# tictacmenthe/F2CNN

Measured on AMD Instinct MI355X. Metric: audio-seconds/sec through filterbank+envelope (HIP, 1 MI355X per rank); the +CNN figure of BASELINE's metric is value_with_cnn / blocks.cfg4, higher is better.
Workload: dtype f64 filter state + f64 utterance FFT + f32 row FFT; 1 GPU; cfg3: filterbank + Hilbert envelope + 50 Hz LPF in one call (f32 FFT), batch of 1000 x 1 s utterances per GPU, 128 channels, ENV1 (float64) out; channels=128, lpf_hz=50, launch_batch=1000, outputs_resident_in_hbm=True, parallelism=utterance-sharded x1, no collective, utterances_sent_back_by_the_accuracy_guard=0

## Files before the change

### f2cnn_amd/csrc/f2_api.hip

```cpp
#include "f2_internal.h"

char g_f2_err[512] = {0};

int f2_fail(f2_ctx* ctx, int code, const char* fmt, ...) {
    char* dst = ctx ? ctx->err : g_f2_err;
    va_list ap;
    va_start(ap, fmt);
    vsnprintf(dst, 512, fmt, ap);
    va_end(ap);
    return code;
}

int f2_reserve(f2_ctx* ctx, f2_scratch& s, size_t bytes) {
    if (bytes <= s.bytes) return F2_OK;
    if (s.ptr) {
        F2_HIP(ctx, hipStreamSynchronize(ctx->stream));
        F2_HIP(ctx, hipFree(s.ptr));
        s.ptr = nullptr;
        s.bytes = 0;
    }
    size_t want = (bytes + 255) & ~size_t(255);
    hipError_t e = hipMalloc(&s.ptr, want);
    if (e != hipSuccess) {
        s.ptr = nullptr;
// ... 170 lines not shown
    }
    *count = n;
    return F2_OK;
}

int f2_ctx_create(int device, f2_ctx** out) {
    if (!out) return f2_fail(nullptr, F2_ERR_INVALID, "ctx out pointer is NULL");
    *out = nullptr;
    int n = 0;
    hipError_t e = hipGetDeviceCount(&n);
    if (e != hipSuccess || n <= 0)
        return f2_fail(nullptr, F2_ERR_HIP, "no HIP device available (%s)",
                       e != hipSuccess ? hipGetErrorString(e) : "device count is 0");
    if (device < 0 || device >= n) return f2_fail(nullptr, F2_ERR_INVALID, "device %d out of range [0,%d)", device, n);
    f2_ctx* ctx = new f2_ctx();
    ctx->device = device;
    e = hipSetDevice(device);
    if (e == hipSuccess) e = hipStreamCreateWithFlags(&ctx->stream, hipStreamNonBlocking);
    hipDeviceProp_t prop;
    if (e == hipSuccess) e = hipGetDeviceProperties(&prop, device);
    if (e == hipSuccess) e = hipHostMalloc((void**)&ctx->host_flags, 64, hipHostMallocDefault);
    if (e != hipSuccess) {
        f2_fail(nullptr, F2_ERR_HIP, "context setup on device %d -> %s", device, hipGetErrorString(e));
        delete ctx;
        return F2_ERR_HIP;
    }
    ctx->num_cus = prop.multiProcessorCount;
    if (strncmp(prop.gcnArchName, "gfx950", 6) != 0) {
        f2_fail(nullptr, F2_ERR_UNSUPPORTED, "device %d is %s; this library is built for gfx950 only", device,
                prop.gcnArchName);
        (void)hipStreamDestroy(ctx->stream);
        (void)hipHostFree(ctx->host_flags);
        delete ctx;
        return F2_ERR_UNSUPPORTED;
    }
    int rc = f2_reserve(ctx, ctx->flags, 64);
    if (rc != F2_OK) {
        memcpy(g_f2_err, ctx->err, sizeof(g_f2_err));
        (void)hipStreamDestroy(ctx->stream);
        (void)hipHostFree(ctx->host_flags);
        delete ctx;
        return rc;
    }
    *out = ctx;
    return F2_OK;
}

int f2_ctx_destroy(f2_ctx* ctx) {
    if (!ctx) return F2_OK;
    (void)hipSetDevice(ctx->device);
    (void)hipStreamSynchronize(ctx->stream);
    f2_scratch* all[] = {&ctx->coefs, &ctx->offsets, &ctx->stage_in, &ctx->stage_out, &ctx->stage_aux,
                         &ctx->work,  &ctx->work2,   &ctx->xbuf,      &ctx->flags,    &ctx->gather_log, &ctx->dense_in,
                         &ctx->stamps, &ctx->noise_wave, &ctx->noise_meta, &ctx->acc_meta, &ctx->score_meta};
    for (f2_scratch* s : all)
        if (s->ptr) (void)hipFree(s->ptr);
    for (auto& v : ctx->prof)
        for (auto& pr : v) {
            (void)hipEventDestroy(pr.first);
            (void)hipEventDestroy(pr.second);
        }
    for (hipEvent_t e : ctx->prof_pool) (void)hipEventDestroy(e);
    for (auto& prec : ctx->tw)
        for (f2_scratch& s : prec)
            if (s.ptr) (void)hipFree(s.ptr);
    for (auto& prec : ctx->tw_large)
        for (f2_scratch& s : prec)
            if (s.ptr) (void)hipFree(s.ptr);
    for (f2_scratch& s : ctx->tw_p3)
        if (s.ptr) (void)hipFree(s.ptr);
    for (f2_scratch& s : ctx->tw_fl)
        if (s.ptr) (void)hipFree(s.ptr);
    for (f2_scratch& s : ctx->tw_split)
        if (s.ptr) (void)hipFree(s.ptr);
    for (f2_scratch* sc : {&ctx->tw_pair[0], &ctx->tw_pair[1], &ctx->pair_list[0], &ctx->pair_list[1]})
        if (sc->ptr) (void)hipFree(sc->ptr);
    if (ctx->work3.ptr) (void)hipFree(ctx->work3.ptr);
    if (ctx->k1_states.ptr) (void)hipFree(ctx->k1_states.ptr);
    if (ctx->k1_mtab.ptr) (void)hipFree(ctx->k1_mtab.ptr);
    if (ctx->k1_order.ptr) (void)hipFree(ctx->k1_order.ptr);
    if (ctx->handoff.ptr) (void)hipFree(ctx->handoff.ptr);
    if (ctx->handoff_off.ptr) (void)hipFree(ctx->handoff_off.ptr);
    for (auto& t : ctx->spec_tabs)
        for (f2_scratch* sc : {&t.hu, &t.e, &t.lgroup, &t.e64})
            if (sc->ptr) (void)hipFree(sc->ptr);
    for (f2_scratch* sc : {&ctx->spec_x, &ctx->spec_rho, &ctx->spec_xpart, &ctx->spec_meta, &ctx->spec_uflag, &ctx->spec_lptab})
        if (sc->ptr) (void)hipFree(sc->ptr);
    for (auto& prec : ctx->tw_sp)
        for (f2_scratch& sc : prec)
            if (sc.ptr) (void)hipFree(sc.ptr);
    for (auto& sp : ctx->up_inflight) (void)hipEventDestroy(sp.done);
    for (auto& b : ctx->up_big) {
        if (b.ptr) (void)hipHostFree(b.ptr);
        (void)hipEventDestroy(b.done);
    }
    if (ctx->up_ring) (void)hipHostFree(ctx->up_ring);
    if (ctx->host_flags) (void)hipHostFree(ctx->host_flags);
    if (ctx->own_stream && ctx->stream) (void)hipStreamDestroy(ctx->stream);
    delete ctx;
    return F2_OK;
}

int f2_ctx_synchronize(f2_ctx* ctx) {
    F2_CHECK(nullptr, ctx, F2_ERR_INVALID, "ctx is NULL");
    F2_HIP(ctx, hipStreamSynchronize(ctx->stream));
    return F2_OK;
}

int f2_ctx_set_stream(f2_ctx* ctx, void* hip_stream) {
    F2_CHECK(nullptr, ctx, F2_ERR_INVALID, "ctx is NULL");
    F2_HIP(ctx, hipStreamSynchronize(ctx->stream));
    if (ctx->own_stream && ctx->stream) F2_HIP(ctx, hipStreamDestroy(ctx->stream));
    if (hip_stream) {
        ctx->stream = (hipStream_t)hip_stream;
        ctx->own_stream = false;
    } else {
        F2_HIP(ctx, hipStreamCreateWithFlags(&ctx->stream, hipStreamNonBlocking));
        ctx->own_stream = true;
    }
    return F2_OK;
}

void* f2_ctx_get_stream(f2_ctx* ctx) { return ctx ? (void*)ctx->stream : nullptr; }

const char* f2_last_error(f2_ctx* ctx) { return ctx ? ctx->err : g_f2_err; }

namespace {
struct opt_entry {
    const char* key;
    int f2_ctx::*ifield;
    float f2_ctx::*ffield;
    double lo, hi;
};
const opt_entry kOptions[] = {
    {"spectral", &f2_ctx::opt_spectral, nullptr, 0, 1},
    {"spectral_tol", nullptr, &f2_ctx::opt_spectral_tol, 0, 1},
    {"spectral_min_rows", &f2_ctx::opt_spectral_min_rows, nullptr, 0, 1 << 30},
    {"spectral_min_pad", &f2_ctx::opt_spectral_min_pad, nullptr, -1, 1 << 16},
    {"spectral_guard_dump", &f2_ctx::opt_spectral_guard_dump, nullptr, 0, 1},
    {"k1_split", &f2_ctx::opt_k1_split, nullptr, -1, 64},
    {"k1_queue", &f2_ctx::opt_k1_queue, nullptr, -1, 1},
    {"k1_qwaves", &f2_ctx::opt_k1_qwaves, nullptr, 0, 1 << 20},
    {"env_pair", &f2_ctx::opt_env_pair, nullptr, 0, 1},
    {"env_plan4", &f2_ctx::opt_env_plan4, nullptr, 0, 1},
    {"cnn_f16x3", &f2_ctx::opt_cnn_f16x3, nullptr, 0, 1},
    {"cnn_bf16x3", &f2_ctx::opt_cnn_f16x3, nullptr, 0, 1},
    {"cnn_ws", &f2_ctx::opt_cnn_ws, nullptr, 0, 1},
    {"cnn_ws_dense", &f2_ctx::opt_cnn_ws_dense, nullptr, 0, 1},
    {"gather_blocked", &f2_ctx::opt_gather_blocked, nullptr, 0, 1},
};
const opt_entry* find_option(const char* key) {
    if (!key) return nullptr;
    for (const opt_entry& e : kOptions)
        if (strcmp(e.key, key) == 0) return &e;
    return nullptr;
}
}

int f2_ctx_set_option(f2_ctx* ctx, const char* key, double value) {
    F2_CHECK(nullptr, ctx, F2_ERR_INVALID, "ctx is NULL");
    const opt_entry* e = find_option(key);
    F2_CHECK(ctx, e, F2_ERR_INVALID, "unknown option '%s'", key ? key : "(null)");
    F2_CHECK(ctx, value >= e->lo && value <= e->hi, F2_ERR_INVALID, "option %s: %g outside [%g, %g]", key, value, e->lo, e->hi);
    if (e->ifield) {
        F2_CHECK(ctx, value == (double)(int)value, F2_ERR_INVALID, "option %s takes an integer", key);
        ctx->*(e->ifield) = (int)value;
    } else {
// ... 475 lines not shown
```

### f2cnn_amd/csrc/f2_internal.h

```cpp
#pragma once
#include <hip/hip_runtime.h>

#include <cstdarg>
#include <cstdint>
#include <cstdio>
#include <cstring>
#include <mutex>
#include <string>
#include <utility>
#include <vector>

#include "../../include/f2cnn_hip.h"

struct f2_scratch {
    void* ptr = nullptr;
    size_t bytes = 0;
};

struct f2_spec_tables {
    int log2h = 0, C = 0;
    std::vector<double> coefs;
    int64_t tpitch = 0;
    f2_scratch hu, e, lgroup, e64;
};
#define F2_SPECTRAL_MIN_LOG2H 12
#define F2_SPECTRAL_MAX_LOG2H 15

struct f2_ctx {
    int device = 0;
    hipStream_t stream = nullptr;
    bool own_stream = true;
    int num_cus = 0;
    char err[512] = {0};
    f2_scratch coefs;
    f2_scratch offsets;
    f2_scratch stage_in;
    f2_scratch stage_out;
    f2_scratch stage_aux;
    f2_scratch work;
    f2_scratch work2;
    f2_scratch xbuf;
    f2_scratch dense_in;
    f2_scratch noise_wave;
    f2_scratch noise_meta;
    f2_scratch acc_meta;
    f2_scratch score_meta;
    f2_scratch gather_log;
    f2_scratch tw[2][16];
    f2_scratch tw_fl[16];
    f2_scratch tw_p3[2];
    f2_scratch tw_large[2][24];
    f2_scratch tw_split[24];
    std::vector<int> pair_list_host[2];
    f2_scratch tw_pair[2], pair_list[2];
    f2_scratch work3;
    f2_scratch handoff, handoff_off;
    std::vector<int64_t> handoff_off_host;
    f2_scratch k1_states, k1_mtab;
    f2_scratch k1_order;
    int k1_mtab_L = 0;
    std::vector<double> k1_mtab_coefs;
    std::vector<int64_t> offsets_host;
    std::vector<double> coefs_host;
    bool prof_on = false;
    struct prof_span {
        hipEvent_t first, second;
        bool closed;
    };
    std::vector<prof_span> prof[F2_K_COUNT];
    std::vector<hipEvent_t> prof_pool;
    std::vector<f2_spec_tables> spec_tabs;
    f2_scratch spec_x, spec_rho;
    f2_scratch spec_xpart;
    f2_scratch spec_meta, spec_uflag;
    f2_scratch spec_gdump;
    size_t spec_gdump_rows = 0;
    std::vector<int> spec_meta_host;
    int spec_coefs_ok = -1;
    int spec_min_pad = 64;
    size_t spec_last_B = 0;
    f2_scratch tw_sp[2][16];
    f2_scratch spec_lptab;
    double spec_lptab_a1 = 0.0;
    int spec_lptab_nt = 0;
    int opt_spectral = 1;
    int opt_spectral_min_rows = 4096;
    float opt_spectral_tol = 4e-6f;
    int opt_spectral_min_pad = -1;
    int opt_spectral_guard_dump = 0;
    int opt_k1_split = -1;
    int opt_k1_queue = -1;
    int opt_k1_qwaves = 0;
    int opt_env_pair = 1;
    int opt_cnn_f16x3 = 1;
    int opt_cnn_ws = 1;
    int opt_cnn_ws_dense = 1;
    int opt_gather_blocked = 1;
    int opt_env_plan4 = 0;
    char* up_ring = nullptr;
    size_t up_cap = 0, up_head = 0;
    struct up_span {
        size_t begin, end;
        hipEvent_t done;
    };
    std::vector<up_span> up_inflight;
    struct up_side {
// ... 221 lines not shown
```

### f2cnn_amd/csrc/f2_spectral.hip

```cpp
#define f2fft f2fft_sp
#undef F2_PLAN13_PASSES
#define F2_PLAN13_PASSES 4
#include <algorithm>
#include <cmath>
#include <complex>
#include <thread>

#include "f2_fft_lds.h"

using namespace f2fft;

namespace {

typedef float f2_f4 __attribute__((ext_vector_type(4)));
constexpr int SPEC_GB = 16;

constexpr int KS_CGROUP = 32;
constexpr int KS_CGROUP_LONG = 8;
constexpr int KS_STORE_AUX = 2;
typedef unsigned int f2_u4 __attribute__((ext_vector_type(4)));
typedef unsigned int f2_u2 __attribute__((ext_vector_type(2)));
__device__ __forceinline__ __amdgpu_buffer_rsrc_t row_buffer(double* y, int n) {
    return __builtin_amdgcn_make_buffer_rsrc(y, 0, n * 8, 0x00020000);
}
// ... 593 lines not shown
    constexpr int D = 1 << LOGD;
    constexpr int NT = threads_for<double, LOG2H>();
    constexpr int H = 1 << LOG2H;
    constexpr int CS = cpad_size(H);
    constexpr int R0 = 1 << plan_bits(LOG2H, 0);
    constexpr int NB0 = H / R0;
    constexpr int ITER0 = (NB0 + NT - 1) / NT;
    constexpr int PT = plan_points_per_thread(LOG2H, NT);
    constexpr bool FULL0 = NB0 % NT == 0;
    __shared__ __attribute__((aligned(16))) cpx<double> lds[CS];
    constexpr int TWL = plan_tw_lds_count(LOG2H);
    __shared__ __attribute__((aligned(16))) cpx<double> twl[TWL > 0 ? TWL : 1];
    const cpx<double>* __restrict__ V = tw + plan_tw_total(LOG2H);
    const int tid = threadIdx.x;
    const int ul = blockIdx.x >> LOGD, ph = blockIdx.x & (D - 1);
    const int b = ulist[ul];
    const int64_t off = offsets[b];
    const int n = (int)(offsets[b + 1] - off);
    const WaveT* __restrict__ x = wave + off;
    for (int i = tid; i < TWL; i += NT) twl[i] = tw[plan_tw_offset(LOG2H, 1) + i];
    cpx<double> v[PT];
#pragma unroll
    for (int i = 0; i < ITER0; ++i) {
        const int bf = tid + i * NT;
        if (FULL0 || bf < NB0) {
#pragma unroll
            for (int j = 0; j < R0; ++j) {
                const int i0 = D * 2 * (bf + j * NB0) + ph, i1 = i0 + D;
                v[i * R0 + j] = {i0 < n ? (double)x[i0] : 0.0, i1 < n ? (double)x[i1] : 0.0};
            }
        }
    }
    fft_all<double, LOG2H, false, PT, NT, false>(lds, tw, twl, tid, v);
    cpx<float>* __restrict__ Xo = X + (size_t)ul * xpitch;
    cpx<double>* __restrict__ Xp = Xpart + (size_t)blockIdx.x * (H + 1);
    for (int k = 1 + tid; k <= H / 2; k += NT) {
        const cpx<double> zk = lds[cpad(k)], zh = lds[cpad(H - k)];
        const cpx<double> e = {0.5 * (zk.re + zh.re), 0.5 * (zk.im - zh.im)};
        const cpx<double> o = {0.5 * (zk.im + zh.im), -0.5 * (zk.re - zh.re)};
        const cpx<double> w = V[k];
        const cpx<double> wo = {o.re * w.re - o.im * w.im, o.re * w.im + o.im * w.re};
        if constexpr (LOGD == 0) {
            Xo[k] = {(float)(e.re + wo.re), (float)(e.im + wo.im)};
            Xo[H - k] = {(float)(e.re - wo.re), (float)(-(e.im - wo.im))};
        } else {
            Xp[k] = {e.re + wo.re, e.im + wo.im};
            Xp[H - k] = {e.re - wo.re, -(e.im - wo.im)};
        }
    }
    if (tid == 0) {
        const cpx<double> z0 = lds[cpad(0)];
        if constexpr (LOGD == 0) {
            Xo[0] = {(float)(z0.re + z0.im), 0.f};
            Xo[H] = {(float)(z0.re - z0.im), 0.f};
        } else {
            Xp[0] = {z0.re + z0.im, 0.0};
            Xp[H] = {z0.re - z0.im, 0.0};
        }
    }
}

template <int LOG2HS, int LOGD>
__global__ __launch_bounds__(256) void k_spectrum_combine(const cpx<double>* __restrict__ Xpart, const cpx<double>* __restrict__ e64,
                                                          cpx<float>* __restrict__ X, int64_t xpitch) {
    constexpr int D = 1 << LOGD, HS = 1 << LOG2HS, H = D * HS, M = 2 * H;
    const int ul = blockIdx.y;
    const int k = blockIdx.x * 256 + threadIdx.x;
    if (k > H) return;
    const int kk = k & (2 * HS - 1);
    double re = 0.0, im = 0.0;
#pragma unroll
    for (int ph = 0; ph < D; ++ph) {
        const cpx<double>* __restrict__ Xp = Xpart + ((size_t)ul * D + ph) * (HS + 1);
        cpx<double> xp = kk <= HS ? Xp[kk] : Xp[2 * HS - kk];
        if (kk > HS) xp.im = -xp.im;
        const cpx<double> w = e64[(ph * k) & (M - 1)];
        re += xp.re * w.re - xp.im * w.im;
        im += xp.re * w.im + xp.im * w.re;
    }
    X[(size_t)ul * xpitch + k] = {(float)re, (float)im};
}

constexpr int TAIL_TB = 32;
constexpr int TAIL_WAVES = 4;

template <typename WaveT>
__global__ __launch_bounds__((64 * TAIL_WAVES)) void k_tail_state(const WaveT* __restrict__ wave, const int64_t* __restrict__ offsets,
                                                                const double* __restrict__ coefs, int C, int groups,
                                                                const int* __restrict__ ulist, int nutt,
                                                                const int* __restrict__ Lgroup, float* __restrict__ rho,
                                                                double two_over_m) {
    __shared__ double xss[TAIL_WAVES][TAIL_TB];
    const int lane = threadIdx.x & 63;
    const int wid = __builtin_amdgcn_readfirstlane(threadIdx.x >> 6);
    const int unit = blockIdx.x * TAIL_WAVES + wid;
    if (unit >= nutt * groups) return;
    const int ul = unit / groups, g = unit - ul * groups;
    const int b = ulist[ul];
    const int64_t off = offsets[b];
    const int64_t N = offsets[b + 1] - off;
    const int cc = g * 64 + lane;
    const int c = min(cc, C - 1);
    const double* k = coefs + (size_t)c * 10;
    const double rB0 = 1.0 / k[6];
    const double b0 = k[0] * rB0, a1 = k[7] * rB0, a2 = k[8] * rB0;
    const double c1 = k[1] / k[0], c2 = k[2] / k[0], c3 = k[3] / k[0], c4 = k[4] / k[0];
    const double scale = (b0 * b0) * (b0 * b0) / k[9] * two_over_m;
    double* xs = xss[wid];
    const WaveT* w = wave + off;
    const int64_t L = min((int64_t)Lgroup[g], N);
    const int64_t nblk = (L + TAIL_TB - 1) / TAIL_TB;
    const int64_t t_begin = N - nblk * TAIL_TB;
    double z10 = 0, z11 = 0, z20 = 0, z21 = 0, z30 = 0, z31 = 0, z40 = 0, z41 = 0;
    auto sample = [&](int64_t t) { return (lane < TAIL_TB && t >= 0 && t < N) ? (double)w[t] : 0.0; };
    double xnext = sample(t_begin + lane);
    for (int64_t t0 = t_begin; t0 < N; t0 += TAIL_TB) {
        if (lane < TAIL_TB) xs[lane] = xnext;
        xnext = sample(t0 + TAIL_TB + lane);
        __builtin_amdgcn_fence(__ATOMIC_RELEASE, "wavefront");
        __builtin_amdgcn_wave_barrier();
        __builtin_amdgcn_fence(__ATOMIC_ACQUIRE, "wavefront");
        double p1 = 0, p2 = 0, p3 = 0;
#pragma unroll
        for (int s2 = 0; s2 < TAIL_TB + 3; ++s2) {
            double n1 = 0, n2 = 0, n3 = 0;
            if (s2 < TAIL_TB) {
                const double wv = fma(-a1, z10, fma(-a2, z11, xs[s2]));
                n1 = fma(c1, z10, wv);
                z11 = z10;
                z10 = wv;
            }
            if (s2 >= 1 && s2 - 1 < TAIL_TB) {
                const double wv = fma(-a1, z20, fma(-a2, z21, p1));
                n2 = fma(c2, z20, wv);
                z21 = z20;
                z20 = wv;
            }
            if (s2 >= 2 && s2 - 2 < TAIL_TB) {
                const double wv = fma(-a1, z30, fma(-a2, z31, p2));
                n3 = fma(c3, z30, wv);
                z31 = z30;
                z30 = wv;
            }
            if (s2 >= 3) {
                const double wv = fma(-a1, z40, fma(-a2, z41, p3));
                z41 = z40;
                z40 = wv;
            }
            p1 = n1;
            p2 = n2;
            p3 = n3;
        }
        __builtin_amdgcn_fence(__ATOMIC_RELEASE, "wavefront");
        __builtin_amdgcn_wave_barrier();
        __builtin_amdgcn_fence(__ATOMIC_ACQUIRE, "wavefront");
    }
    const double ia2 = 1.0 / a2;
    const double R10 = (a1 - c1) * z10 + a2 * z11, R11 = a2 * z10 + c1 * a2 * z11;
    const double R20 = (a1 - c2) * z20 + a2 * z21, R21 = a2 * z20 + c2 * a2 * z21;
    const double R30 = (a1 - c3) * z30 + a2 * z31, R31 = a2 * z30 + c3 * a2 * z31;
    const double R40 = (a1 - c4) * z40 + a2 * z41, R41 = a2 * z40 + c4 * a2 * z41;
    double d0[2], d1[2], d2[2], d3[2];
    d3[0] = R40;
    d3[1] = R41;
    {
        const double p0 = R30, p1q = R31 + c4 * R30, p2q = c4 * R31;
        const double q = p2q * ia2;
        d2[0] = p0 - q;
        d2[1] = p1q - q * a1;
        d3[0] += q;
    }
    {
        const double s0 = 1.0, s1 = c4 + c3, s2 = c4 * c3;
        double p0 = s0 * R20, p1q = s0 * R21 + s1 * R20, p2q = s1 * R21 + s2 * R20, p3q = s2 * R21;
        const double q1 = p3q * ia2;
        p2q -= q1 * a1;
        p1q -= q1;
        const double q0 = p2q * ia2;
        p1q -= q0 * a1;
        p0 -= q0;
        d1[0] = p0;
        d1[1] = p1q;
        d2[0] += q0;
        d2[1] += q1;
    }
    {
        const double s0 = 1.0, s1 = c4 + c3, s2 = c4 * c3;
        const double t0 = s0, t1 = s1 + c2 * s0, t2 = s2 + c2 * s1, t3 = c2 * s2;
        double p0 = t0 * R10, p1q = t0 * R11 + t1 * R10, p2q = t1 * R11 + t2 * R10, p3q = t2 * R11 + t3 * R10, p4q = t3 * R11;
        const double q2 = p4q * ia2;
        p3q -= q2 * a1;
        p2q -= q2;
        const double q1 = p3q * ia2;
        p2q -= q1 * a1;
        p1q -= q1;
        const double q0 = p2q * ia2;
        p1q -= q0 * a1;
        p0 -= q0;
        d0[0] = p0;
        d0[1] = p1q;
        const double qq = q2 * ia2;
        d1[0] += q0 - qq;
        d1[1] += q1 - qq * a1;
        d2[0] += qq;
    }
    if (cc < C) {
        float* r = rho + ((size_t)ul * C + cc) * 8;
        typedef float f4 __attribute__((ext_vector_type(4)));
        *reinterpret_cast<f4*>(r) = f4{(float)(d0[0] * scale), (float)(d0[1] * scale), (float)(d1[0] * scale), (float)(d1[1] * scale)};
        *reinterpret_cast<f4*>(r + 4) = f4{(float)(d2[0] * scale), (float)(d2[1] * scale), (float)(d3[0] * scale), (float)(d3[1] * scale)};
    }
}

__global__ __launch_bounds__(256) void k_spectral_tables(const double* __restrict__ coefs, int C, int H, int64_t tpitch,
                                                         f2_f4* __restrict__ hu, cpx<float>* __restrict__ e,
                                                         cpx<double>* __restrict__ e64) {
    const int M = 2 * H;
    const int64_t q = (int64_t)blockIdx.x * 256 + threadIdx.x;
    const int c = blockIdx.y;
    double sn, cs;
    sincospi(2.0 * (double)q / (double)M, &sn, &cs);
    const double wr = cs, wi = -sn;
    if (c == C) {
        if (q < M) {
            e[q] = {(float)wr, (float)wi};
            if (e64) e64[q] = {wr, wi};
        }
        return;
    }
    if (q >= tpitch) return;
    f2_f4 out = {0.f, 0.f, 0.f, 0.f};
    if (q <= H) {
        const double* k = coefs + (size_t)c * 10;
        const double rB0 = 1.0 / k[6];
        const double b0 = k[0] * rB0, a1 = k[7] * rB0, a2 = k[8] * rB0;
        const double s = (b0 * b0) * (b0 * b0) / k[9] * (2.0 / M);
        const double w2r = wr * wr - wi * wi, w2i = 2.0 * wr * wi;
        const double dr = 1.0 + a1 * wr + a2 * w2r, di = a1 * wi + a2 * w2i;
        const double dn = 1.0 / (dr * dr + di * di);
        const double ur = dr * dn, ui = -di * dn;
        double hr = s, hi = 0.0;
#pragma unroll
        for (int m = 0; m < 4; ++m) {
            const double cm = k[1 + m] / k[0];
            const double nr = 1.0 + cm * wr, ni = cm * wi;
            const double tr = nr * ur - ni * ui, ti = nr * ui + ni * ur;
            const double xr = hr * tr - hi * ti, xi = hr * ti + hi * tr;
            hr = xr;
            hi = xi;
        }
        out = {(float)hr, (float)hi, (float)ur, (float)ui};
    }
    hu[(size_t)c * tpitch + q] = out;
}

int64_t ringing_length(double a1, double a2, double tol, int64_t limit) {
    if (!(a2 > 1e-3 && a2 < 1.0) || a1 * a1 >= 4.0 * a2) return 0;
    const double lr = 0.5 * std::log(a2);
    const double np = std::max(1.0, -3.0 / lr);
    const double target = std::log(tol) + 3.0 * std::log(np) + np * lr;
    double lo = np, hi = np;
    while (3.0 * std::log(hi) + hi * lr > target) {
        hi *= 2;
        if (hi > (double)limit) return 0;
    }
    for (int it = 0; it < 60; ++it) {
        const double mid = 0.5 * (lo + hi);
        if (3.0 * std::log(mid) + mid * lr > target) lo = mid;
        else hi = mid;
    }
    return (int64_t)std::ceil(hi) + 64;
}

}

bool f2_spectral_supports_len(int64_t n, int min_pad) {
    if (n < 2) return false;
    const int log2h = f2_log2_ceil(n) - 1;
    if (log2h < F2_SPECTRAL_MIN_LOG2H || log2h > F2_SPECTRAL_MAX_LOG2H) return false;
    return (int64_t(2) << log2h) - n >= std::max(64, min_pad);
}

bool f2_spectral_supports_coefs(const std::vector<double>& coefs, int C, std::vector<int>* Lgroup, int* min_pad) {
    if (coefs.size() != (size_t)C * 10 || C <= 0) return false;
    const int groups = (C + 63) / 64;
    if (Lgroup) Lgroup->assign((size_t)groups, 0);
    double peak = 0.0;
    for (int c = 0; c < C; ++c) {
        const double* k = &coefs[(size_t)c * 10];
        if (k[5] != 0.0 || k[0] == 0.0 || k[6] == 0.0 || k[9] == 0.0) return false;
        for (int q = 0; q < 10; ++q)
            if (!std::isfinite(k[q])) return false;
        const int64_t L = ringing_length(k[7] / k[6], k[8] / k[6], 1e-8, int64_t(1) << 17);
        if (L <= 0) return false;
        if (Lgroup) (*Lgroup)[(size_t)c / 64] = std::max((*Lgroup)[(size_t)c / 64], (int)L);
        peak = std::max(peak, 3.0 / (-0.5 * std::log(k[8] / k[6])));
    }
    if (min_pad) *min_pad = ((int)std::ceil(1.1 * peak) + 31) / 32 * 32;
    return true;
}

static int spectral_tables(f2_ctx* ctx, const double* d_coefs, int C, int log2h, f2_spec_tables** out) {
    for (auto& t : ctx->spec_tabs)
        if (t.log2h == log2h && t.C == C && t.coefs == ctx->coefs_host) {
            *out = &t;
            return F2_OK;
        }
    if (ctx->spec_tabs.size() >= 6) {
        F2_HIP(ctx, hipStreamSynchronize(ctx->stream));
        for (f2_scratch* s : {&ctx->spec_tabs.front().hu, &ctx->spec_tabs.front().e, &ctx->spec_tabs.front().lgroup,
                              &ctx->spec_tabs.front().e64})
            if (s->ptr) (void)hipFree(s->ptr);
        ctx->spec_tabs.erase(ctx->spec_tabs.begin());
    }
    f2_spec_tables t;
    t.log2h = log2h;
    t.C = C;
    t.coefs = ctx->coefs_host;
    std::vector<int> Lg;
    if (!f2_spectral_supports_coefs(t.coefs, C, &Lg, nullptr)) return f2_fail(ctx, F2_ERR_INVALID, "coefficient table not eligible");
    const int H = 1 << log2h, M = 2 * H;
    t.tpitch = H + 8;
    F2_TRY(f2_reserve(ctx, t.hu, sizeof(float) * 4 * (size_t)C * (size_t)t.tpitch));
    F2_TRY(f2_reserve(ctx, t.e, sizeof(float) * 2 * (size_t)M));
    F2_TRY(f2_reserve(ctx, t.lgroup, sizeof(int) * Lg.size()));
    if (log2h > 13) F2_TRY(f2_reserve(ctx, t.e64, sizeof(double) * 2 * (size_t)M));
    hipLaunchKernelGGL(k_spectral_tables, dim3((unsigned)((M + 255) / 256), (unsigned)(C + 1)), dim3(256), 0, ctx->stream, d_coefs, C, H,
                       t.tpitch, (f2_f4*)t.hu.ptr, (cpx<float>*)t.e.ptr, (cpx<double>*)t.e64.ptr);
    F2_HIP(ctx, hipGetLastError());
    F2_TRY(f2_upload_async(ctx, t.lgroup.ptr, Lg.data(), sizeof(int) * Lg.size()));
    ctx->spec_tabs.push_back(std::move(t));
    *out = &ctx->spec_tabs.back();
    return F2_OK;
}

static int lowpass_table(f2_ctx* ctx, double a1, double b0, int nt, int sp, LowpassConsts* K, const f2_f4** d_tab) {
    const long double q = -(long double)a1;
    K->qf = (float)q;
    K->b0f = (float)b0;
    K->g1 = (float)powl(q, sp);
    K->g2 = (float)powl(q, 2 * sp);
    K->g4 = (float)powl(q, 4 * sp);
    K->g8 = (float)powl(q, 8 * sp);
    K->gw = (double)powl(q, 64 * sp);
    K->gblk = (double)powl(q, sp * nt);
    f2_scratch& slot = ctx->spec_lptab;
    double& slot_a1 = ctx->spec_lptab_a1;
    *d_tab = (const f2_f4*)slot.ptr;
    constexpr int TMAX = 1024;
    if (slot.ptr && slot_a1 == a1) return F2_OK;
    std::vector<float> tab((size_t)TMAX * 4);
    for (int t = 0; t < TMAX; ++t) {
        const int lane = t & 63;
        tab[4 * (size_t)t] = (float)powl(q, sp * (lane + 1));
        tab[4 * (size_t)t + 1] = (float)powl(q, sp * t);
        tab[4 * (size_t)t + 2] = (float)powl(q, sp * ((lane & 15) + 1));
        tab[4 * (size_t)t + 3] = (float)powl(q, sp * ((lane & 31) + 1));
    }
    F2_TRY(f2_reserve(ctx, slot, sizeof(float) * tab.size()));
    F2_TRY(f2_upload_async(ctx, slot.ptr, tab.data(), sizeof(float) * tab.size()));
    slot_a1 = a1;
    *d_tab = (const f2_f4*)slot.ptr;
    return F2_OK;
}

template <typename WaveT, int LOG2H>
static int launch_group(f2_ctx* ctx, const WaveT* d_wave, const int64_t* d_offsets, const double* d_coefs, int C,
                        const int* d_ulist, int nutt, int64_t min_n, int lpf, double b0, double a1, double* d_env, int* d_uflag,
                        float tol, cpx<float>* d_X, float* d_rho) {
    constexpr int H = 1 << LOG2H, M = 2 * H;
    f2_spec_tables* tab = nullptr;
    F2_TRY(spectral_tables(ctx, d_coefs, C, LOG2H, &tab));
    constexpr int LOGD = LOG2H > 13 ? LOG2H - 13 : 0, LOG2HS = LOG2H - LOGD;
    constexpr int FFTLOG = LOG2H == 15 ? 14 : LOG2H;
    F2_TRY(ensure_twiddles<double>(ctx, LOG2HS, ctx->tw_sp[1][LOG2HS]));
    F2_TRY(ensure_twiddles<float>(ctx, FFTLOG, ctx->tw_sp[0][FFTLOG]));
    const int64_t xpitch = H + 8;
    const int groups = (C + 63) / 64;
    F2_TRY(f2_prof_begin(ctx, F2_K_SPECTRUM));
    cpx<double>* d_part = nullptr;
    if constexpr (LOGD > 0) {
        F2_TRY(f2_reserve(ctx, ctx->spec_xpart, sizeof(double) * 2 * ((size_t)(1 << LOG2HS) + 1) * (size_t)nutt << LOGD));
        d_part = (cpx<double>*)ctx->spec_xpart.ptr;
    }
    hipLaunchKernelGGL((k_utterance_spectrum<WaveT, LOG2HS, LOGD>), dim3((unsigned)nutt << LOGD), dim3(threads_for<double, LOG2HS>()),
                       0, ctx->stream, d_wave, d_offsets, d_ulist, d_X, xpitch, d_part,
                       (const cpx<double>*)ctx->tw_sp[1][LOG2HS].ptr);
    F2_HIP(ctx, hipGetLastError());
    if constexpr (LOGD > 0) {
        hipLaunchKernelGGL((k_spectrum_combine<LOG2HS, LOGD>), dim3((unsigned)((H + 256) / 256), (unsigned)nutt), dim3(256), 0,
                           ctx->stream, (const cpx<double>*)d_part, (const cpx<double>*)tab->e64.ptr, d_X, xpitch);
        F2_HIP(ctx, hipGetLastError());
    }
    F2_TRY(f2_prof_end(ctx, F2_K_SPECTRUM));
    F2_TRY(f2_prof_begin(ctx, F2_K_TAIL));
    const int units = nutt * groups;
    hipLaunchKernelGGL((k_tail_state<WaveT>), dim3((unsigned)((units + TAIL_WAVES - 1) / TAIL_WAVES)), dim3(64 * TAIL_WAVES), 0,
                       ctx->stream, d_wave, d_offsets, d_coefs, C, groups, d_ulist, nutt, (const int*)tab->lgroup.ptr, d_rho,
                       2.0 / M);
    F2_HIP(ctx, hipGetLastError());
    F2_TRY(f2_prof_end(ctx, F2_K_TAIL));
    SpecParams P;
    P.xpitch = xpitch;
    P.tpitch = tab->tpitch;
    P.env = d_env;
    P.uflag = d_uflag;
    P.C = C;
    P.nutt = nutt;
    P.lpf = lpf;
    const f2_f4* d_lptab = nullptr;
    F2_TRY(lowpass_table(ctx, a1, b0, threads_for<float, FFTLOG>(), 2, &P.lp, &d_lptab));
    P.tol = tol;
    P.gdump = ctx->opt_spectral_guard_dump ? (float*)ctx->spec_gdump.ptr : nullptr;
    P.stamps = nullptr;
#ifdef F2_STAMPS
    F2_TRY(f2_stamps_buffer(ctx, (size_t)nutt * C, 8, &P.stamps));
#endif
    F2_TRY(f2_prof_begin(ctx, F2_K_FUSED));
    if constexpr (LOG2H == 15)
        hipLaunchKernelGGL(k_spectral_envelope_long, dim3((unsigned)((size_t)nutt * C)), dim3(threads_for<float, FFTLOG>()), 0,
                           ctx->stream, P, (const cpx<float>*)d_X, (const f2_f4*)tab->hu.ptr, (const cpx<float>*)tab->e.ptr,
                           (const float*)d_rho, d_offsets, d_ulist, d_lptab, (const cpx<float>*)ctx->tw_sp[0][FFTLOG].ptr);
    else if (min_n >= 15 * (M / 16))
        hipLaunchKernelGGL((k_spectral_envelope<FFTLOG, true>), dim3((unsigned)((size_t)nutt * C)), dim3(threads_for<float, FFTLOG>()), 0,
                           ctx->stream, P, (const cpx<float>*)d_X, (const f2_f4*)tab->hu.ptr, (const cpx<float>*)tab->e.ptr,
                           (const float*)d_rho, d_offsets, d_ulist, d_lptab, (const cpx<float>*)ctx->tw_sp[0][FFTLOG].ptr);
    else
        hipLaunchKernelGGL((k_spectral_envelope<FFTLOG, false>), dim3((unsigned)((size_t)nutt * C)), dim3(threads_for<float, FFTLOG>()), 0,
                           ctx->stream, P, (const cpx<float>*)d_X, (const f2_f4*)tab->hu.ptr, (const cpx<float>*)tab->e.ptr,
                           (const float*)d_rho, d_offsets, d_ulist, d_lptab, (const cpx<float>*)ctx->tw_sp[0][FFTLOG].ptr);
    F2_HIP(ctx, hipGetLastError());
    F2_TRY(f2_prof_end(ctx, F2_K_FUSED));
#ifdef F2_STAMPS
    static const char* names_s[8] = {"", "bin 0 ready", "bin 7 ready", "bin 15 ready", "transform inputs", "both transforms + even magnitudes", "odd magnitudes + guard", "lpf+stores"};
    static const char* names_l[8] = {"", "spectrum r=0,2", "transforms r=0,2 + parking", "spectrum r=1,3", "transforms r=1,3 + parking", "low-pass sweep 0", "low-pass sweep 1", "flag"};
    F2_TRY(f2_stamps_report(ctx, P.stamps, (size_t)nutt * C, 8, LOG2H == 15 ? names_l : names_s, "[stamps KS]",
                            "mean ticks (10 ns) per workgroup:", true));
#endif
    return F2_OK;
}

int f2_launch_spectral(f2_ctx* ctx, const void* d_wave, int wave_dtype, const int64_t* d_offsets, const double* d_coefs,
                       int C, const int* d_ulist, int nutt, int64_t min_n, int log2h, int lpf, double cutoff_hz, double* d_env,
                       int* d_uflag) {
    if (nutt <= 0) return F2_OK;
    const double k = lpf ? tan(3.14159265358979323846 * cutoff_hz / 16000.0) : 0.0;
    const double b0 = k / (1.0 + k), a1 = (k - 1.0) / (k + 1.0);
    const float tol = ctx->opt_spectral_tol;
    const int H = 1 << log2h;
    F2_TRY(f2_reserve(ctx, ctx->spec_x, sizeof(float) * 2 * (size_t)(H + 8) * (size_t)nutt));
    F2_TRY(f2_reserve(ctx, ctx->spec_rho, sizeof(float) * 8 * (size_t)nutt * (size_t)C));
    cpx<float>* d_X = (cpx<float>*)ctx->spec_x.ptr;
    float* d_rho = (float*)ctx->spec_rho.ptr;
#define F2_SPEC_CASE(L)                                                                                                          \
    case L:                                                                                                                      \
        return wave_dtype == F2_WAVE_I16                                                                                         \
                   ? launch_group<int16_t, L>(ctx, (const int16_t*)d_wave, d_offsets, d_coefs, C, d_ulist, nutt, min_n, lpf, b0, \
                                              a1, d_env, d_uflag, tol, d_X, d_rho)                                              \
                   : launch_group<double, L>(ctx, (const double*)d_wave, d_offsets, d_coefs, C, d_ulist, nutt, min_n, lpf, b0,   \
                                             a1, d_env, d_uflag, tol, d_X, d_rho);
    switch (log2h) {
        F2_SPEC_CASE(12)
        F2_SPEC_CASE(13)
        F2_SPEC_CASE(14)
        F2_SPEC_CASE(15)
        default:
            return f2_fail(ctx, F2_ERR_UNSUPPORTED, "spectral path: length class 2^%d not built", log2h + 1);
    }
#undef F2_SPEC_CASE
}
```

Before: 203,600 audio-seconds/s.

## Split tail-state IIR recurrence into parallel segments combined via state-transition matrices

The tail-state kernel previously ran one wave per 64-channel group per utterance, serially filtering the full ringing length. Now each wave processes 16 channels across 4 utterances, and long ringing tails are cut into up to 8 segments run by separate waves. The segment end states are combined in LDS using host-precomputed 8x8 transition matrices A^S for each channel. A host bin-packing plan balances segment lengths across waves in a workgroup. This shortens the serial dependency chain and raises parallelism. The costs are extra LDS, a __syncthreads, the per-channel matrix combine, and a permutation search when tables are built.

```diff
diff --git a/f2cnn_amd/csrc/f2_api.hip b/f2cnn_amd/csrc/f2_api.hip
--- a/f2cnn_amd/csrc/f2_api.hip
+++ b/f2cnn_amd/csrc/f2_api.hip
@@ -276,7 +276,7 @@
     if (ctx->handoff.ptr) (void)hipFree(ctx->handoff.ptr);
     if (ctx->handoff_off.ptr) (void)hipFree(ctx->handoff_off.ptr);
     for (auto& t : ctx->spec_tabs)
-        for (f2_scratch* sc : {&t.hu, &t.e, &t.lgroup, &t.e64})
+        for (f2_scratch* sc : {&t.hu, &t.e, &t.tail_units, &t.tail_as, &t.e64})
             if (sc->ptr) (void)hipFree(sc->ptr);
     for (f2_scratch* sc : {&ctx->spec_x, &ctx->spec_rho, &ctx->spec_xpart, &ctx->spec_meta, &ctx->spec_uflag, &ctx->spec_lptab})
         if (sc->ptr) (void)hipFree(sc->ptr);
diff --git a/f2cnn_amd/csrc/f2_internal.h b/f2cnn_amd/csrc/f2_internal.h
--- a/f2cnn_amd/csrc/f2_internal.h
+++ b/f2cnn_amd/csrc/f2_internal.h
@@ -21,7 +21,9 @@
     int log2h = 0, C = 0;
     std::vector<double> coefs;
     int64_t tpitch = 0;
-    f2_scratch hu, e, lgroup, e64;
+    f2_scratch hu, e, e64;
+    f2_scratch tail_units, tail_as;
+    int tail_w = 0, tail_wgq = 0;
 };
 #define F2_SPECTRAL_MIN_LOG2H 12
 #define F2_SPECTRAL_MAX_LOG2H 15
diff --git a/f2cnn_amd/csrc/f2_spectral.hip b/f2cnn_amd/csrc/f2_spectral.hip
--- a/f2cnn_amd/csrc/f2_spectral.hip
+++ b/f2cnn_amd/csrc/f2_spectral.hip
@@ -699,41 +699,63 @@
 }
 
 constexpr int TAIL_TB = 32;
-constexpr int TAIL_WAVES = 4;
+constexpr int TAIL_CG = 16;
+constexpr int TAIL_UQ = 4;
+constexpr int TAIL_SEG = 512;
+constexpr int TAIL_MINW = 4;
+constexpr int TAIL_MAXW = 8;
+constexpr int TAIL_XS = TAIL_UQ * TAIL_TB;
+constexpr int TAIL_ZB = 8 * 64;
+
+struct TailUnit {
+    int g;
+    int seg;
+    int nseg;
+    int S;
+};
 
 template <typename WaveT>
-__global__ __launch_bounds__((64 * TAIL_WAVES)) void k_tail_state(const WaveT* __restrict__ wave, const int64_t* __restrict__ offsets,
-                                                                const double* __restrict__ coefs, int C, int groups,
-                                                                const int* __restrict__ ulist, int nutt,
-                                                                const int* __restrict__ Lgroup, float* __restrict__ rho,
-                                                                double two_over_m) {
-    __shared__ double xss[TAIL_WAVES][TAIL_TB];
+__global__ __launch_bounds__((64 * TAIL_MAXW), 4) void k_tail_state(const WaveT* __restrict__ wave, const int64_t* __restrict__ offsets,
+                                                               const double* __restrict__ coefs, int C,
+                                                               const int* __restrict__ ulist, int nutt,
+                                                               const TailUnit* __restrict__ units, int quads,
+                                                               const double* __restrict__ AS, float* __restrict__ rho,
+                                                               double two_over_m) {
+    extern __shared__ __attribute__((aligned(16))) double tail_lds[];
+    const int W = blockDim.x >> 6;
     const int lane = threadIdx.x & 63;
     const int wid = __builtin_amdgcn_readfirstlane(threadIdx.x >> 6);
-    const int unit = blockIdx.x * TAIL_WAVES + wid;
-    if (unit >= nutt * groups) return;
-    const int ul = unit / groups, g = unit - ul * groups;
-    const int b = ulist[ul];
+    const int j = blockIdx.x / quads, quad = blockIdx.x - j * quads;
+    const TailUnit u = units[j * W + wid];
+    const int g = u.g, seg = u.seg, nseg = u.nseg & 255, S = u.S;
+    const bool meet = (u.nseg & 256) != 0;
+    const int q = lane >> 4, li = lane & 15;
+    const int ul = quad * TAIL_UQ + q;
+    const bool live = g >= 0 && ul < nutt;
+    const int b = ulist[min(ul, nutt - 1)];
     const int64_t off = offsets[b];
-    const int64_t N = offsets[b + 1] - off;
-    const int cc = g * 64 + lane;
+    const int64_t N = live ? offsets[b + 1] - off : 0;
+    const int cc = max(g, 0) * TAIL_CG + li;
     const int c = min(cc, C - 1);
     const double* k = coefs + (size_t)c * 10;
     const double rB0 = 1.0 / k[6];
     const double b0 = k[0] * rB0, a1 = k[7] * rB0, a2 = k[8] * rB0;
     const double c1 = k[1] / k[0], c2 = k[2] / k[0], c3 = k[3] / k[0], c4 = k[4] / k[0];
     const double scale = (b0 * b0) * (b0 * b0) / k[9] * two_over_m;
-    double* xs = xss[wid];
+    double* xs = tail_lds + wid * TAIL_XS;
+    const double* xq = xs + q * TAIL_TB;
+    double* zb = tail_lds + W * TAIL_XS;
     const WaveT* w = wave + off;
-    const int64_t L = min((int64_t)Lgroup[g], N);
-    const int64_t nblk = (L + TAIL_TB - 1) / TAIL_TB;
-    const int64_t t_begin = N - nblk * TAIL_TB;
+    const int64_t t_begin = N - (int64_t)(nseg - seg) * S;
     double z10 = 0, z11 = 0, z20 = 0, z21 = 0, z30 = 0, z31 = 0, z40 = 0, z41 = 0;
-    auto sample = [&](int64_t t) { return (lane < TAIL_TB && t >= 0 && t < N) ? (double)w[t] : 0.0; };
-    double xnext = sample(t_begin + lane);
-    for (int64_t t0 = t_begin; t0 < N; t0 += TAIL_TB) {
-        if (lane < TAIL_TB) xs[lane] = xnext;
-        xnext = sample(t0 + TAIL_TB + lane);
+    auto sample = [&](int64_t t) { return (t >= 0 && t < N) ? (double)w[t] : 0.0; };
+    double xn0 = sample(t_begin + li), xn1 = sample(t_begin + 16 + li);
+    for (int blk = 0; blk < S / TAIL_TB; ++blk) {
+        const int64_t t0 = t_begin + (int64_t)blk * TAIL_TB;
+        xs[q * TAIL_TB + li] = xn0;
+        xs[q * TAIL_TB + 16 + li] = xn1;
+        xn0 = sample(t0 + TAIL_TB + li);
+        xn1 = sample(t0 + TAIL_TB + 16 + li);
         __builtin_amdgcn_fence(__ATOMIC_RELEASE, "wavefront");
         __builtin_amdgcn_wave_barrier();
         __builtin_amdgcn_fence(__ATOMIC_ACQUIRE, "wavefront");
@@ -742,7 +764,7 @@
         for (int s2 = 0; s2 < TAIL_TB + 3; ++s2) {
             double n1 = 0, n2 = 0, n3 = 0;
             if (s2 < TAIL_TB) {
-                const double wv = fma(-a1, z10, fma(-a2, z11, xs[s2]));
+                const double wv = fma(-a1, z10, fma(-a2, z11, xq[s2]));
                 n1 = fma(c1, z10, wv);
                 z11 = z10;
                 z10 = wv;
@@ -771,6 +793,40 @@
         __builtin_amdgcn_fence(__ATOMIC_RELEASE, "wavefront");
         __builtin_amdgcn_wave_barrier();
         __builtin_amdgcn_fence(__ATOMIC_ACQUIRE, "wavefront");
+    }
+    if (meet) {
+        if (seg < nseg - 1) {
+            double* z = zb + (size_t)wid * TAIL_ZB + lane;
+            z[0 * 64] = z10, z[1 * 64] = z11, z[2 * 64] = z20, z[3 * 64] = z21;
+            z[4 * 64] = z30, z[5 * 64] = z31, z[6 * 64] = z40, z[7 * 64] = z41;
+        }
+        __syncthreads();
+    }
+    if (g < 0 || seg != nseg - 1) return;
+    if (nseg > 1) {
+        const double* __restrict__ A = AS + (size_t)c * 64;
+        const double own[8] = {z10, z11, z20, z21, z30, z31, z40, z41};
+        const double* z0 = zb + (size_t)(wid - seg) * TAIL_ZB + lane;
+        double* sl = zb + (size_t)wid * TAIL_ZB + lane;
+        double acc[8];
+#pragma unroll
+        for (int i = 0; i < 8; ++i) acc[i] = z0[i * 64];
+#pragma unroll 1
+        for (int kk = 1; kk < nseg; ++kk) {
+            const double* zk = z0 + (size_t)kk * TAIL_ZB;
+#pragma unroll
+            for (int i = 0; i < 8; ++i) {
+                sl[i * 64] = acc[i];
+                acc[i] = kk < nseg - 1 ? zk[i * 64] : own[i];
+            }
+#pragma unroll 1
+            for (int jj = 0; jj < 8; ++jj) {
+                const double sj = sl[jj * 64];
+#pragma unroll
+                for (int i = 0; i < 8; ++i) acc[i] = fma(A[jj * 8 + i], sj, acc[i]);
+            }
+        }
+        z10 = acc[0], z11 = acc[1], z20 = acc[2], z21 = acc[3], z30 = acc[4], z31 = acc[5], z40 = acc[6], z41 = acc[7];
     }
     const double ia2 = 1.0 / a2;
     const double R10 = (a1 - c1) * z10 + a2 * z11, R11 = a2 * z10 + c1 * a2 * z11;
@@ -821,7 +877,7 @@
         d1[1] += q1 - qq * a1;
         d2[0] += qq;
     }
-    if (cc < C) {
+    if (live && cc < C) {
         float* r = rho + ((size_t)ul * C + cc) * 8;
         typedef float f4 __attribute__((ext_vector_type(4)));
         *reinterpret_cast<f4*>(r) = f4{(float)(d0[0] * scale), (float)(d0[1] * scale), (float)(d1[0] * scale), (float)(d1[1] * scale)};
@@ -900,7 +956,7 @@
 
 bool f2_spectral_supports_coefs(const std::vector<double>& coefs, int C, std::vector<int>* Lgroup, int* min_pad) {
     if (coefs.size() != (size_t)C * 10 || C <= 0) return false;
-    const int groups = (C + 63) / 64;
+    const int groups = (C + TAIL_CG - 1) / TAIL_CG;
     if (Lgroup) Lgroup->assign((size_t)groups, 0);
     double peak = 0.0;
     for (int c = 0; c < C; ++c) {
@@ -910,11 +966,113 @@
             if (!std::isfinite(k[q])) return false;
         const int64_t L = ringing_length(k[7] / k[6], k[8] / k[6], 1e-8, int64_t(1) << 17);
         if (L <= 0) return false;
-        if (Lgroup) (*Lgroup)[(size_t)c / 64] = std::max((*Lgroup)[(size_t)c / 64], (int)L);
+        if (Lgroup) (*Lgroup)[(size_t)c / TAIL_CG] = std::max((*Lgroup)[(size_t)c / TAIL_CG], (int)L);
         peak = std::max(peak, 3.0 / (-0.5 * std::log(k[8] / k[6])));
     }
     if (min_pad) *min_pad = ((int)std::ceil(1.1 * peak) + 31) / 32 * 32;
     return true;
+}
+
+static void tail_plan(const std::vector<double>& coefs, int C, const std::vector<int>& Lg, std::vector<TailUnit>* units, int* W,
+                      int* wgq, std::vector<double>* AS) {
+    const int groups = (int)Lg.size();
+    std::vector<int> nseg((size_t)groups), S((size_t)groups), order((size_t)groups);
+    int total = 0, most = 1;
+    for (int g = 0; g < groups; ++g) {
+        nseg[(size_t)g] = std::min(TAIL_MAXW, std::max(1, (Lg[(size_t)g] + TAIL_SEG - 1) / TAIL_SEG));
+        S[(size_t)g] = ((Lg[(size_t)g] + nseg[(size_t)g] - 1) / nseg[(size_t)g] + TAIL_TB - 1) / TAIL_TB * TAIL_TB;
+        total += nseg[(size_t)g];
+        most = std::max(most, nseg[(size_t)g]);
+        order[(size_t)g] = g;
+    }
+    *W = std::max(most, std::min(TAIL_MINW, total));
+    std::stable_sort(order.begin(), order.end(), [&](int a, int b) { return nseg[(size_t)a] > nseg[(size_t)b]; });
+    std::vector<std::vector<int>> bins;
+    std::vector<int> used;
+    for (int g : order) {
+        size_t j = 0;
+        while (j < used.size() && used[j] + nseg[(size_t)g] > *W) ++j;
+        if (j == used.size()) {
+            used.push_back(0);
+            bins.emplace_back();
+        }
+        bins[j].push_back(g);
+        used[j] += nseg[(size_t)g];
+    }
+    units->assign(bins.size() * (size_t)*W, TailUnit{-1, 0, 0, 0});
+    std::vector<int64_t> load((size_t)*W, 0);
+    for (size_t j = 0; j < bins.size(); ++j) {
+        std::vector<int> perm = bins[j], best;
+        std::sort(perm.begin(), perm.end());
+        int64_t best_peak = INT64_MAX;
+        int tried = 0;
+        do {
+            for (int lead = 0; lead <= *W - used[j]; ++lead) {
+                std::vector<int64_t> l = load;
+                int slot = lead;
+                for (int g : perm)
+                    for (int k = 0; k < nseg[(size_t)g]; ++k) l[(size_t)slot++] += S[(size_t)g];
+                const int64_t peak = *std::max_element(l.begin(), l.end());
+                if (peak < best_peak) {
+                    best_peak = peak;
+                    best = perm;
+                    best.push_back(lead);
+                }
+            }
+        } while (std::next_permutation(perm.begin(), perm.end()) && ++tried < 5040);
+        int slot = best.back();
+        best.pop_back();
+        for (int g : best)
+            for (int k = 0; k < nseg[(size_t)g]; ++k) {
+                load[(size_t)slot] += S[(size_t)g];
+                (*units)[j * (size_t)*W + (size_t)slot++] = TailUnit{g, k, nseg[(size_t)g], S[(size_t)g]};
+            }
+    }
+    *wgq = (int)used.size();
+    for (size_t j = 0; j < used.size(); ++j) {
+        bool meet = false;
+        for (int i = 0; i < *W; ++i) meet = meet || (*units)[j * (size_t)*W + (size_t)i].nseg > 1;
+        if (meet)
+            for (int i = 0; i < *W; ++i) (*units)[j * (size_t)*W + (size_t)i].nseg |= 256;
+    }
+    AS->assign((size_t)C * 64, 0.0);
+    auto mul = [](const double* a, const double* b, double* o) {
+        for (int i = 0; i < 8; ++i)
+            for (int j = 0; j < 8; ++j) {
+                double acc = 0.0;
+                for (int m = 0; m < 8; ++m) acc += a[i * 8 + m] * b[m * 8 + j];
+                o[i * 8 + j] = acc;
+            }
+    };
+    for (int c = 0; c < C; ++c) {
+        const int g = c / TAIL_CG;
+        if (nseg[(size_t)g] < 2) continue;
+        const double* k = &coefs[(size_t)c * 10];
+        const double rB0 = 1.0 / k[6], a1 = k[7] * rB0, a2 = k[8] * rB0;
+        double A[64] = {0}, P[64] = {0}, T[64];
+        double in[8] = {0};
+        for (int m = 0; m < 4; ++m) {
+            double* r = A + (2 * m) * 8;
+            for (int j = 0; j < 8; ++j) r[j] = in[j];
+            r[2 * m] -= a1;
+            r[2 * m + 1] -= a2;
+            A[(2 * m + 1) * 8 + 2 * m] = 1.0;
+            const double cm = k[1 + m] / k[0];
+            for (int j = 0; j < 8; ++j) in[j] = r[j];
+            in[2 * m] += cm;
+        }
+        for (int i = 0; i < 8; ++i) P[i * 9] = 1.0;
+        for (int e = S[(size_t)g]; e > 0; e >>= 1) {
+            if (e & 1) {
+                mul(P, A, T);
+                std::copy(T, T + 64, P);
+            }
+            mul(A, A, T);
+            std::copy(T, T + 64, A);
+        }
+        for (int i = 0; i < 8; ++i)
+            for (int j = 0; j < 8; ++j) (*AS)[(size_t)c * 64 + (size_t)j * 8 + (size_t)i] = P[i * 8 + j];
+    }
 }
 
 static int spectral_tables(f2_ctx* ctx, const double* d_coefs, int C, int log2h, f2_spec_tables** out) {
@@ -925,8 +1083,8 @@
         }
     if (ctx->spec_tabs.size() >= 6) {
         F2_HIP(ctx, hipStreamSynchronize(ctx->stream));
-        for (f2_scratch* s : {&ctx->spec_tabs.front().hu, &ctx->spec_tabs.front().e, &ctx->spec_tabs.front().lgroup,
-                              &ctx->spec_tabs.front().e64})
+        for (f2_scratch* s : {&ctx->spec_tabs.front().hu, &ctx->spec_tabs.front().e, &ctx->spec_tabs.front().tail_units,
+                              &ctx->spec_tabs.front().tail_as, &ctx->spec_tabs.front().e64})
             if (s->ptr) (void)hipFree(s->ptr);
         ctx->spec_tabs.erase(ctx->spec_tabs.begin());
     }
@@ -940,12 +1098,17 @@
     t.tpitch = H + 8;
     F2_TRY(f2_reserve(ctx, t.hu, sizeof(float) * 4 * (size_t)C * (size_t)t.tpitch));
     F2_TRY(f2_reserve(ctx, t.e, sizeof(float) * 2 * (size_t)M));
-    F2_TRY(f2_reserve(ctx, t.lgroup, sizeof(int) * Lg.size()));
+    std::vector<TailUnit> units;
+    std::vector<double> AS;
+    tail_plan(t.coefs, C, Lg, &units, &t.tail_w, &t.tail_wgq, &AS);
+    F2_TRY(f2_reserve(ctx, t.tail_units, sizeof(TailUnit) * units.size()));
+    F2_TRY(f2_reserve(ctx, t.tail_as, sizeof(double) * AS.size()));
     if (log2h > 13) F2_TRY(f2_reserve(ctx, t.e64, sizeof(double) * 2 * (size_t)M));
     hipLaunchKernelGGL(k_spectral_tables, dim3((unsigned)((M + 255) / 256), (unsigned)(C + 1)), dim3(256), 0, ctx->stream, d_coefs, C, H,
                        t.tpitch, (f2_f4*)t.hu.ptr, (cpx<float>*)t.e.ptr, (cpx<double>*)t.e64.ptr);
     F2_HIP(ctx, hipGetLastError());
-    F2_TRY(f2_upload_async(ctx, t.lgroup.ptr, Lg.data(), sizeof(int) * Lg.size()));
+    F2_TRY(f2_upload_async(ctx, t.tail_units.ptr, units.data(), sizeof(TailUnit) * units.size()));
+    F2_TRY(f2_upload_async(ctx, t.tail_as.ptr, AS.data(), sizeof(double) * AS.size()));
     ctx->spec_tabs.push_back(std::move(t));
     *out = &ctx->spec_tabs.back();
     return F2_OK;
@@ -993,7 +1156,6 @@
     F2_TRY(ensure_twiddles<double>(ctx, LOG2HS, ctx->tw_sp[1][LOG2HS]));
     F2_TRY(ensure_twiddles<float>(ctx, FFTLOG, ctx->tw_sp[0][FFTLOG]));
     const int64_t xpitch = H + 8;
-    const int groups = (C + 63) / 64;
     F2_TRY(f2_prof_begin(ctx, F2_K_SPECTRUM));
     cpx<double>* d_part = nullptr;
     if constexpr (LOGD > 0) {
@@ -1011,10 +1173,10 @@
     }
     F2_TRY(f2_prof_end(ctx, F2_K_SPECTRUM));
     F2_TRY(f2_prof_begin(ctx, F2_K_TAIL));
-    const int units = nutt * groups;
-    hipLaunchKernelGGL((k_tail_state<WaveT>), dim3((unsigned)((units + TAIL_WAVES - 1) / TAIL_WAVES)), dim3(64 * TAIL_WAVES), 0,
-                       ctx->stream, d_wave, d_offsets, d_coefs, C, groups, d_ulist, nutt, (const int*)tab->lgroup.ptr, d_rho,
-                       2.0 / M);
+    const int quads = (nutt + TAIL_UQ - 1) / TAIL_UQ;
+    hipLaunchKernelGGL((k_tail_state<WaveT>), dim3((unsigned)quads * (unsigned)tab->tail_wgq), dim3(64 * (unsigned)tab->tail_w),
+                       sizeof(double) * (size_t)tab->tail_w * (TAIL_XS + TAIL_ZB), ctx->stream, d_wave, d_offsets, d_coefs, C, d_ulist,
+                       nutt, (const TailUnit*)tab->tail_units.ptr, quads, (const double*)tab->tail_as.ptr, d_rho, 2.0 / M);
     F2_HIP(ctx, hipGetLastError());
     F2_TRY(f2_prof_end(ctx, F2_K_TAIL));
     SpecParams P;
```

After: 205,400 audio-seconds/s (median of 6 runs). No clear change (+0.8%).
